# ArchieGertsman/spark-sched-sim

Hardware: AMD Instinct MI355X
Metric: env-steps/sec at 4096 batched envs (TPC-H, 10 exec) (higher is better)
Workload: dtype int64+f64

## Files before the change

include/sss.h:

```cpp
#ifndef SSS_H
#define SSS_H
#include <stddef.h>
#include <stdint.h>

#ifdef __cplusplus
extern "C" {
#endif

typedef struct sss_handle sss_handle;

typedef struct sss_cfg {
  int32_t num_executors;
  int32_t job_arrival_cap;
  int32_t max_jobs;
  int32_t reserved;
  double job_arrival_rate;
  double moving_delay;
  double warmup_delay;
  double beta;
} sss_cfg;

typedef struct sss_dims {
  int32_t num_envs, num_executors, job_cap, stage_stride;
  int32_t node_cap;
// ... 24 lines not shown
  SSS_E_STALLED = 5,
  SSS_E_NO_DURATION = 6,
  SSS_E_INVARIANT = 7,
  SSS_E_NEED_RESET = 8,
  SSS_E_NO_LIMIT = 9,
  SSS_E_CAPACITY = 10
};

int sss_query_dims(const sss_cfg* cfg, const void* pack, size_t pack_bytes, int num_envs, sss_dims* out);

int sss_create(const sss_cfg* cfg, const void* pack, size_t pack_bytes, int num_envs, int device, sss_handle** out);

int sss_bind_buffers(sss_handle* h, const sss_buffers* buffers);

int sss_reset(sss_handle* h, const uint64_t* seeds_dev, const double* time_limits_dev, const uint8_t* mask_dev, void* stream);

#define SSS_SKIP_ENV (-2147483647 - 1)
int sss_step(sss_handle* h, const int32_t* stage_idx_dev, const int32_t* num_exec_dev, int auto_reset, uint64_t seed_stride, void* stream);

int sss_step_bounded(sss_handle* h, const int32_t* stage_idx_dev, const int32_t* num_exec_dev, int auto_reset, uint64_t seed_stride, int max_events,
                     uint8_t* ready_dev, void* stream);

int sss_policy(sss_handle* h, int policy, int param, int32_t* stage_idx_dev, int32_t* num_exec_dev, void* stream);

int sss_rollout(sss_handle* h, int policy, int param, int n_steps, int auto_reset, uint64_t seed_stride, void* stream);

typedef struct sss_decima_graph {
  const uint8_t* active_dev;
  const int64_t* node_off_dev;
  const int64_t* job_off_dev;
  const int64_t* edge_off_dev;
  float num_tasks_scale;
  float work_scale;
  float* x_dev;
  int64_t* node_obs_dev;
  int64_t* node_loc_dev;
  int64_t* node_job_dev;
  int64_t* sched_rank_dev;
  int32_t* gen_dev;
  uint32_t* node_recv_dev;
  uint8_t* stage_mask_dev;
  int64_t* src_dev;
  int64_t* dst_dev;
  int64_t* edge_obs_dev;
  uint32_t* edge_layers_dev;
  int64_t* job_obs_dev;
// ... 333 lines not shown
```

spark_sched_sim_amd/binding.py:

```python
from __future__ import annotations

import ctypes as C
import os.path as osp

CSRC = osp.join(osp.dirname(osp.abspath(__file__)), "csrc")
LIB_NAME = "libsss_hip.so"


class SssCfg(C.Structure):
    _fields_ = [("num_executors", C.c_int32), ("job_arrival_cap", C.c_int32), ("max_jobs", C.c_int32),
                ("reserved", C.c_int32), ("job_arrival_rate", C.c_double), ("moving_delay", C.c_double),
                ("warmup_delay", C.c_double), ("beta", C.c_double)]


class SssDims(C.Structure):
    _fields_ = [("num_envs", C.c_int32), ("num_executors", C.c_int32), ("job_cap", C.c_int32),
                ("stage_stride", C.c_int32), ("node_cap", C.c_int32), ("edge_cap", C.c_int32),
                ("obs_i32", C.c_int32), ("obs_f64", C.c_int32), ("state_bytes", C.c_int64),
                ("env_stride", C.c_int64), ("off_t_arrival", C.c_int64), ("off_t_completed", C.c_int64),
                ("off_jobs", C.c_int64), ("off_active", C.c_int64), ("off_dur_ring", C.c_int64),
                ("job_rec_bytes", C.c_int32), ("hdr_bytes", C.c_int32)]


class SssBuffers(C.Structure):
# ... 109 lines not shown
    _fields_ = [("bits_dev", C.c_void_p), ("n", C.c_int64), ("n_layers", C.c_int32), ("chunk", C.c_int32), ("n_chunks", C.c_int32), ("phase", C.c_int32),
                ("cnt_dev", C.c_void_p), ("off_dev", C.c_void_p), ("base", C.c_int64 * 32), ("out_dev", C.c_void_p)]


class SssReturnsArgs(C.Structure):
    _fields_ = [("T", C.c_int64), ("B", C.c_int64), ("active_dev", C.c_void_p), ("t_before_dev", C.c_void_p), ("t_after_dev", C.c_void_p), ("rewards_dev", C.c_void_p),
                ("beta", C.c_double), ("out_dev", C.c_void_p)]


class SssBaselineArgs(C.Structure):
    _fields_ = [("T", C.c_int64), ("B", C.c_int64), ("R", C.c_int32), ("skip_empty", C.c_int32), ("active_dev", C.c_void_p), ("times_dev", C.c_void_p),
                ("values_dev", C.c_void_p), ("n_dev", C.c_void_p), ("out_dev", C.c_void_p)]


class SssArenaArray(C.Structure):
    _fields_ = [("src_dev", C.c_void_p), ("dst_dev", C.c_void_p), ("elem_bytes", C.c_int32), ("per_row", C.c_int32), ("kind", C.c_int32), ("shift", C.c_int32)]


class SssArenaArgs(C.Structure):
    _fields_ = [("n_arrays", C.c_int32), ("n_obs", C.c_int32), ("totals_dev", C.c_void_p), ("cursor_dev", C.c_void_p), ("capacity", C.c_int64 * 4),
                ("rows_hint", C.c_int64), ("arrays", SssArenaArray * 24)]


EXPORTS = ["sss_query_dims", "sss_create", "sss_bind_buffers", "sss_reset", "sss_step", "sss_step_bounded", "sss_policy", "sss_rollout",
           "sss_decima_graph_build", "sss_decima_layer_lists", "sss_prefix_rows", "sss_decima_policy", "sss_decima_sample", "sss_gnn_launch",
           "sss_linear_wgrad_scratch", "sss_linear_wgrad", "sss_mlp_supported", "sss_mlp_recompute_supported", "sss_mlp_split_supported", "sss_mlp_forward", "sss_mlp_backward", "sss_mlp_wgrad_scratch", "sss_mlp_backward_wgrad", "sss_mlp_wgrad_finish", "sss_collect_step", "sss_gnn_encode", "sss_rows_op", "sss_rows_concat", "sss_segment_categorical", "sss_bit_lists", "sss_arena_append", "sss_discounted_returns", "sss_sequence_baselines", "sss_last_error", "sss_destroy", "sss_abi_sizeof"]
POLICY_IDS = {"fair": 0, "fifo": 1, "hash": 2, "wfair": 3, "sjfcp": 4}
WFAIR_ALPHA_RANGE = (-4, 4)
ABI_STRUCTS = {"sss_cfg": SssCfg, "sss_dims": SssDims, "sss_buffers": SssBuffers, "sss_decima_graph": SssDecimaGraph, "sss_decima_lists": SssDecimaLists,
               "sss_bit_list_args": SssBitListArgs, "sss_gnn_args": SssGnnArgs, "sss_decima_policy_args": SssDecimaPolicyArgs,
               "sss_decima_sample_args": SssDecimaSampleArgs, "sss_gnn_encode_args": SssGnnEncodeArgs, "sss_collect_args": SssCollectArgs,
               "sss_mlp_args": SssMlpArgs, "sss_arena_array": SssArenaArray, "sss_arena_args": SssArenaArgs, "sss_returns_args": SssReturnsArgs,
               "sss_baseline_args": SssBaselineArgs, "sss_rows_args": SssRowsArgs, "sss_concat_part": SssConcatPart, "sss_concat_args": SssConcatArgs, "sss_segcat_args": SssSegcatArgs}


def load_library(path: str | None = None) -> C.CDLL:
    path = path or osp.join(CSRC, LIB_NAME)
    if not osp.exists(path):
        raise RuntimeError(
            f"{path} not found: the HIP extension has not been built "
            "(run `python -c 'import __graft_entry__ as g; g.build()'` or spark_sched_sim_amd/build.py). "
            "There is no CPU fallback.")
    return C.CDLL(path)


class Binding:
    def __init__(self, lib: C.CDLL | None = None):
        self.lib = lib if lib is not None else load_library()
        L = self.lib
        L.sss_query_dims.argtypes = [C.POINTER(SssCfg), C.c_void_p, C.c_size_t, C.c_int, C.POINTER(SssDims)]
        L.sss_create.argtypes = [C.POINTER(SssCfg), C.c_void_p, C.c_size_t, C.c_int, C.c_int, C.POINTER(C.c_void_p)]
        L.sss_bind_buffers.argtypes = [C.c_void_p, C.POINTER(SssBuffers)]
        L.sss_reset.argtypes = [C.c_void_p, C.c_void_p, C.c_void_p, C.c_void_p, C.c_void_p]
        L.sss_step.argtypes = [C.c_void_p, C.c_void_p, C.c_void_p, C.c_int, C.c_uint64, C.c_void_p]
        L.sss_step_bounded.argtypes = [C.c_void_p, C.c_void_p, C.c_void_p, C.c_int, C.c_uint64, C.c_int, C.c_void_p, C.c_void_p]
        L.sss_policy.argtypes = [C.c_void_p, C.c_int, C.c_int, C.c_void_p, C.c_void_p, C.c_void_p]
        L.sss_rollout.argtypes = [C.c_void_p, C.c_int, C.c_int, C.c_int, C.c_int, C.c_uint64, C.c_void_p]
        L.sss_decima_graph_build.argtypes = [C.c_void_p, C.POINTER(SssDecimaGraph), C.c_void_p]
        L.sss_decima_layer_lists.argtypes = [C.c_int, C.POINTER(SssDecimaLists), C.c_void_p]
        L.sss_prefix_rows.argtypes = [C.c_void_p, C.c_int64, C.c_int64, C.c_void_p, C.c_int, C.c_int, C.c_void_p, C.c_void_p, C.c_void_p, C.c_void_p]
        L.sss_decima_policy.argtypes = [C.c_void_p, C.POINTER(SssDecimaPolicyArgs), C.c_void_p]
        L.sss_decima_sample.argtypes = [C.c_int, C.c_int, C.POINTER(SssDecimaSampleArgs), C.c_void_p]
        L.sss_gnn_launch.argtypes = [C.c_int, C.POINTER(SssGnnArgs), C.c_void_p]
        L.sss_linear_wgrad_scratch.argtypes = [C.c_int, C.c_int]
        L.sss_linear_wgrad_scratch.restype = C.c_int64
        L.sss_linear_wgrad.argtypes = [C.c_void_p, C.c_int64, C.c_void_p, C.c_int64, C.c_int64, C.c_int, C.c_int, C.c_void_p, C.c_void_p, C.c_void_p, C.c_void_p]
        L.sss_gnn_encode.argtypes = [C.POINTER(SssGnnEncodeArgs), C.c_void_p]
        L.sss_collect_step.argtypes = [C.POINTER(SssCollectArgs), C.c_int, C.c_void_p]
        L.sss_mlp_supported.argtypes = [C.c_int] * 5
        L.sss_mlp_recompute_supported.argtypes = [C.c_int]
        L.sss_mlp_split_supported.argtypes = [C.c_int]
        L.sss_mlp_forward.argtypes = [C.POINTER(SssMlpArgs), C.c_void_p]
        L.sss_mlp_backward.argtypes = [C.POINTER(SssMlpArgs), C.c_void_p]
        L.sss_mlp_wgrad_scratch.argtypes = [C.c_int]
        L.sss_mlp_wgrad_scratch.restype = C.c_int64
        L.sss_mlp_backward_wgrad.argtypes = [C.POINTER(SssMlpArgs), C.c_void_p, C.c_void_p]
        L.sss_mlp_wgrad_finish.argtypes = [C.c_int] + [C.c_void_p] * 8
        L.sss_discounted_returns.argtypes = [C.POINTER(SssReturnsArgs), C.c_void_p]
        L.sss_sequence_baselines.argtypes = [C.POINTER(SssBaselineArgs), C.c_void_p]
        L.sss_bit_lists.argtypes = [C.POINTER(SssBitListArgs), C.c_void_p]
# ... 1 lines not shown
        L.sss_rows_op.argtypes = [C.POINTER(SssRowsArgs), C.c_void_p]
        L.sss_rows_concat.argtypes = [C.POINTER(SssConcatArgs), C.c_void_p]
        L.sss_segment_categorical.argtypes = [C.POINTER(SssSegcatArgs), C.c_int, C.c_void_p]
        L.sss_last_error.restype = C.c_char_p
        L.sss_destroy.argtypes = [C.c_void_p]
        L.sss_abi_sizeof.argtypes = [C.c_char_p]
        self.check_abi()

    def check_abi(self) -> None:
        bad = [(name, C.sizeof(cls), self.lib.sss_abi_sizeof(name.encode())) for name, cls in ABI_STRUCTS.items()
               if C.sizeof(cls) != self.lib.sss_abi_sizeof(name.encode())]
        if bad:
            raise RuntimeError("binding / library mismatch (struct, sizeof in binding.py, sizeof in the library): " + ", ".join(map(str, bad)))

    def check(self, rc: int) -> None:
        if rc != 0:
            raise ValueError(f"sss error {rc}: {self.lib.sss_last_error().decode()}")

    def query_dims(self, cfg: SssCfg, pack: bytes, num_envs: int) -> SssDims:
        d = SssDims()
        self.check(self.lib.sss_query_dims(C.byref(cfg), pack, len(pack), num_envs, C.byref(d)))
        return d

    def create(self, cfg: SssCfg, pack: bytes, num_envs: int, device: int) -> C.c_void_p:
        h = C.c_void_p()
        self.check(self.lib.sss_create(C.byref(cfg), pack, len(pack), num_envs, device, C.byref(h)))
        return h


def device_of(dev):
    import contextlib

    import torch
    dev = torch.device(dev)
    return torch.cuda.device(dev) if dev.type == "cuda" else contextlib.nullcontext()
```

spark_sched_sim_amd/csrc/sss_hip_sim.hip:

```cpp
#include <hip/hip_runtime.h>

#include "sss_sim.h"
#include "sss_narrow.h"

int sss_narrow_hot_bytes() { return (int)sizeof(SssHot); }
int sss_narrow_static_lds_bytes() { return SSS_STATIC_LDS_BYTES; }

int sss_narrow_launch_reset(const SssKernelArgs& a, int num_envs, const uint64_t* seeds, const double* tl, const uint8_t* mask, void* stream) {
  hipLaunchKernelGGL(sss_reset_kernel, dim3(num_envs), dim3(64), (size_t)a.P.pool_bytes, (hipStream_t)stream, a, seeds, tl, mask);
  return (int)hipGetLastError();
}
int sss_narrow_launch_step_bounded(const SssKernelArgs& a, int num_envs, const int32_t* stage_idx, const int32_t* num_exec, int auto_reset, uint64_t seed_stride,
                                   int budget, uint8_t* ready, void* stream) {
  hipLaunchKernelGGL(sss_step_bounded_kernel, dim3(num_envs), dim3(64), (size_t)a.P.pool_bytes, (hipStream_t)stream, a, stage_idx, num_exec, auto_reset, seed_stride,
                     budget, ready);
  return (int)hipGetLastError();
}
int sss_narrow_launch_step(const SssKernelArgs& a, int num_envs, const int32_t* stage_idx, const int32_t* num_exec, int auto_reset, uint64_t seed_stride,
                           void* stream) {
  hipLaunchKernelGGL(sss_step_kernel, dim3(num_envs), dim3(64), (size_t)a.P.pool_bytes, (hipStream_t)stream, a, stage_idx, num_exec, auto_reset, seed_stride);
  return (int)hipGetLastError();
}
int sss_narrow_launch_policy(const SssKernelArgs& a, int num_envs, int policy, int param, int32_t* stage_idx, int32_t* num_exec, void* stream) {
  hipLaunchKernelGGL(sss_policy_kernel, dim3(num_envs), dim3(64), (size_t)a.P.pool_bytes, (hipStream_t)stream, a, policy, param, stage_idx, num_exec);
  return (int)hipGetLastError();
}
int sss_narrow_launch_rollout(const SssKernelArgs& a, int num_envs, int policy, int param, int n_steps, int auto_reset, uint64_t seed_stride, void* stream) {
  if (policy >= SSS_POLICY_WFAIR)
    hipLaunchKernelGGL(sss_rollout_heur_kernel, dim3(num_envs), dim3(64), (size_t)a.P.pool_bytes, (hipStream_t)stream, a, policy, param, n_steps, auto_reset, seed_stride);
  else
    hipLaunchKernelGGL(sss_rollout_kernel, dim3(num_envs), dim3(64), (size_t)a.P.pool_bytes, (hipStream_t)stream, a, policy, param, n_steps, auto_reset, seed_stride);
  return (int)hipGetLastError();
}

#ifdef SSS_EVPROF3
extern "C" int sss_debug_prof(unsigned long long* out64) {
  if (hipMemcpyFromSymbol(out64, HIP_SYMBOL(g_prof3), sizeof(unsigned long long) * 96) != hipSuccess) return -1;
  static const unsigned long long zeros[96] = {0};
  return hipMemcpyToSymbol(HIP_SYMBOL(g_prof3), zeros, sizeof(zeros)) == hipSuccess ? 0 : -1;
}
extern "C" int sss_debug_prof_min(unsigned long long min_step_ticks) {
  return hipMemcpyToSymbol(HIP_SYMBOL(g_prof3_min), &min_step_ticks, sizeof(min_step_ticks)) == hipSuccess ? 0 : -1;
}
// ... 2 lines not shown
```

spark_sched_sim_amd/csrc/sss_hip_wide.hip:

```cpp
#define SSS_WIDE 1
#include <hip/hip_runtime.h>

#include "sss_sim.h"
#include "sss_wide.h"

int sss_wide_hot_bytes() { return (int)sizeof(SssHot); }
int sss_wide_static_lds_bytes() { return SSS_STATIC_LDS_BYTES; }

int sss_wide_launch_reset(const SssKernelArgs& a, int num_envs, const uint64_t* seeds, const double* tl, const uint8_t* mask, void* stream) {
  hipLaunchKernelGGL(sss_reset_kernel_wide, dim3(num_envs), dim3(64), (size_t)a.P.pool_bytes, (hipStream_t)stream, a, seeds, tl, mask);
  return (int)hipGetLastError();
}
int sss_wide_launch_step_bounded(const SssKernelArgs& a, int num_envs, const int32_t* stage_idx, const int32_t* num_exec, int auto_reset, uint64_t seed_stride,
                                 int budget, uint8_t* ready, void* stream) {
  hipLaunchKernelGGL(sss_step_bounded_kernel_wide, dim3(num_envs), dim3(64), (size_t)a.P.pool_bytes, (hipStream_t)stream, a, stage_idx, num_exec, auto_reset,
                     seed_stride, budget, ready);
  return (int)hipGetLastError();
}
int sss_wide_launch_step(const SssKernelArgs& a, int num_envs, const int32_t* stage_idx, const int32_t* num_exec, int auto_reset, uint64_t seed_stride,
                         void* stream) {
  hipLaunchKernelGGL(sss_step_kernel_wide, dim3(num_envs), dim3(64), (size_t)a.P.pool_bytes, (hipStream_t)stream, a, stage_idx, num_exec, auto_reset, seed_stride);
  return (int)hipGetLastError();
}
int sss_wide_launch_policy(const SssKernelArgs& a, int num_envs, int policy, int param, int32_t* stage_idx, int32_t* num_exec, void* stream) {
  hipLaunchKernelGGL(sss_policy_kernel_wide, dim3(num_envs), dim3(64), (size_t)a.P.pool_bytes, (hipStream_t)stream, a, policy, param, stage_idx, num_exec);
  return (int)hipGetLastError();
}
int sss_wide_launch_rollout(const SssKernelArgs& a, int num_envs, int policy, int param, int n_steps, int auto_reset, uint64_t seed_stride, void* stream) {
  if (policy >= SSS_POLICY_WFAIR)
    hipLaunchKernelGGL(sss_rollout_heur_kernel_wide, dim3(num_envs), dim3(64), (size_t)a.P.pool_bytes, (hipStream_t)stream, a, policy, param, n_steps, auto_reset, seed_stride);
  else
    hipLaunchKernelGGL(sss_rollout_kernel_wide, dim3(num_envs), dim3(64), (size_t)a.P.pool_bytes, (hipStream_t)stream, a, policy, param, n_steps, auto_reset, seed_stride);
  return (int)hipGetLastError();
}

#ifdef SSS_EVPROF3
extern "C" int sss_debug_prof_wide(unsigned long long* out64) {
  if (hipMemcpyFromSymbol(out64, HIP_SYMBOL(g_prof3), sizeof(unsigned long long) * 96) != hipSuccess) return -1;
  static const unsigned long long zeros[96] = {0};
  return hipMemcpyToSymbol(HIP_SYMBOL(g_prof3), zeros, sizeof(zeros)) == hipSuccess ? 0 : -1;
}
extern "C" int sss_debug_prof_min_wide(unsigned long long min_step_ticks) {
  return hipMemcpyToSymbol(HIP_SYMBOL(g_prof3_min), &min_step_ticks, sizeof(min_step_ticks)) == hipSuccess ? 0 : -1;
}
#endif
```

spark_sched_sim_amd/csrc/sss_host.h:

```cpp
#pragma once
#include <math.h>
#include <stdio.h>
#include <stdlib.h>
#include <string.h>

#include <string>
#include <vector>

#include "../../include/sss.h"
#include "sss_layout.h"
#include "sss_train.h"
#include "sss_rows.h"
#include "sss_narrow.h"
#include "sss_wide.h"

static bool sss_is_wide(int num_executors) { return num_executors > 64; }
static int sss_hot_bytes(int num_executors) { return sss_is_wide(num_executors) ? sss_wide_hot_bytes() : sss_narrow_hot_bytes(); }

static thread_local std::string g_sss_err;
static int sss_fail(int code, const std::string& msg) {
  g_sss_err = msg;
  return code;
}

// ... 60 lines not shown
      }
      if (!moved) break;
    }
    for (int i = 0; i < n; i++) best = dist[i] > best ? dist[i] : best;
  }
  return best;
}

struct sss_handle {
  sss_cfg cfg;
  SssPackHost ph;
  int max_dag_depth;
  SssLayout L;
  SssBuffers B;
  bool bound;
  int device;
  void* pack_dev;
  void* zig_dev;
  void* eff_dev;
  void* jump_dev;
  void* common_dev;
  SssParams P;
  SssPackDev pk;
};

static int sss_validate(const sss_cfg* cfg, const void* pack, size_t pack_bytes, int num_envs, SssPackHost* ph, int* J_cap) {
  if (!cfg) return sss_fail(-1, "cfg is NULL");
  if (int prc = sss_pack_parse((const uint8_t*)pack, pack_bytes, ph))
    return sss_fail(-2, prc == -2   ? "workload pack: a stage has a negative task count (a count beyond int32 wrapped when the pack was written)"
                        : prc == -3 ? "workload pack: negative task duration (a duration beyond int32 milliseconds wrapped when the pack was written, or the trace set holds one)"
                        : prc == -4 ? "workload pack: a duration list descriptor points outside the duration pool or holds 2^30 or more entries"
                                    : "workload pack is malformed (expected SSSPACK2, n_queries x n_sizes templates, <= 64 stages/job, <= 255 edges/job, <= 16 executor levels)");
  if (num_envs < 1) return sss_fail(-3, "num_envs must be >= 1");
  if (cfg->num_executors < 1 || cfg->num_executors > SSS_MAX_EXEC_ANY) return sss_fail(-4, "num_executors must be in [1, 128]");
  int cap = cfg->job_arrival_cap > 0 ? cfg->job_arrival_cap : 0;
  int jc = cfg->max_jobs > 0 ? cfg->max_jobs : cap;
  if (jc <= 0) return sss_fail(-5, "max_jobs is required when job_arrival_cap is None");
  if (cap > jc) return sss_fail(-5, "max_jobs is smaller than job_arrival_cap");
  if (jc > SSS_MAX_JOBS) return sss_fail(-5, "job capacity above 1024 is not supported by this build");
  if (!(cfg->job_arrival_rate > 0)) return sss_fail(-6, "job_arrival_rate must be > 0");
  if (!(cfg->beta >= 0)) return sss_fail(-6, "beta must be >= 0");
  *J_cap = jc;
  return 0;
}

static std::vector<int32_t> sss_build_eff(const uint8_t* pack, const SssPackHost& ph, const int8_t lvl_of[8], double warmup_delay) {
  const uint32_t* keymask = (const uint32_t*)(pack + ph.sec_off[7]);
// ... 239 lines not shown
    return sss_fail(-13, "copying the duration descriptors to the device failed");
  }
  std::vector<uint8_t> common = sss_build_common_pool(cfg->num_executors);
  h->common_dev = be_alloc(common.size());
  if (!h->common_dev || be_h2d(h->common_dev, common.data(), common.size())) {
    sss_destroy(h);
    return sss_fail(-11, "device allocation failed");
  }
  pk.eff = (const int32_t*)h->eff_dev;
  pk.eff0 = pk.eff + (size_t)ph.total_stages * 8 * 3 * 4;
  pk.pcg_jump = (const uint64_t*)h->jump_dev;
  pk.lvl_thr = (const uint64_t*)h->jump_dev + jump_words;
  pk.common_pool = (const uint8_t*)h->common_dev;
  h->pk = pk;
  *out = h;
  return 0;
}

extern "C" int sss_bind_buffers(sss_handle* h, const sss_buffers* b) {
  if (!h || !b) return sss_fail(-1, "NULL argument");
  if (!b->state_dev || !b->nodes_dev || !b->edge_links_dev || !b->dag_ptr_dev || !b->exec_supplies_dev || !b->obs_i32_dev || !b->obs_f64_dev)
    return sss_fail(-20, "every buffer in sss_buffers must be provided");
  if (((uintptr_t)b->state_dev) & 255) return sss_fail(-21, "state_dev must be 256-byte aligned");
  h->B.state = b->state_dev, h->B.nodes = b->nodes_dev, h->B.edge_links = b->edge_links_dev, h->B.dag_ptr = b->dag_ptr_dev;
  h->B.exec_supplies = b->exec_supplies_dev, h->B.obs_i32 = b->obs_i32_dev, h->B.obs_f64 = b->obs_f64_dev;
  h->B.gen = h->bound ? h->B.gen + 1 : 1, h->B.gen_pad = 0;
  h->bound = true;
  return 0;
}

static SssKernelArgs sss_args(const sss_handle* h) {
  SssKernelArgs a;
  a.L = h->L, a.B = h->B, a.P = h->P, a.pk = h->pk;
  return a;
}

extern "C" int sss_reset(sss_handle* h, const uint64_t* seeds_dev, const double* time_limits_dev, const uint8_t* mask_dev, void* stream) {
  if (!h || !seeds_dev) return sss_fail(-1, "NULL argument");
  if (!h->bound) return sss_fail(-22, "sss_bind_buffers has not been called");
  BeDeviceGuard guard(h->device);
  const SssKernelArgs ka = sss_args(h);
  if (int rc = sss_is_wide(h->L.E) ? sss_wide_launch_reset(ka, h->L.num_envs, seeds_dev, time_limits_dev, mask_dev, stream)
                                   : be_launch_reset(ka, h->L.num_envs, seeds_dev, time_limits_dev, mask_dev, stream)) return sss_fail(-30, std::string("reset launch failed: ") + be_error(rc));
  return 0;
}

extern "C" int sss_step(sss_handle* h, const int32_t* stage_idx_dev, const int32_t* num_exec_dev, int auto_reset, uint64_t seed_stride, void* stream) {
  if (!h || !stage_idx_dev || !num_exec_dev) return sss_fail(-1, "NULL argument");
  if (!h->bound) return sss_fail(-22, "sss_bind_buffers has not been called");
  BeDeviceGuard guard(h->device);
  const SssKernelArgs ka = sss_args(h);
  if (int rc = sss_is_wide(h->L.E) ? sss_wide_launch_step(ka, h->L.num_envs, stage_idx_dev, num_exec_dev, auto_reset, seed_stride, stream)
                                   : be_launch_step(ka, h->L.num_envs, stage_idx_dev, num_exec_dev, auto_reset, seed_stride, stream)) return sss_fail(-30, std::string("step launch failed: ") + be_error(rc));
  return 0;
}

extern "C" int sss_step_bounded(sss_handle* h, const int32_t* stage_idx_dev, const int32_t* num_exec_dev, int auto_reset, uint64_t seed_stride, int max_events,
                                uint8_t* ready_dev, void* stream) {
  if (!h || !stage_idx_dev || !num_exec_dev || !ready_dev) return sss_fail(-1, "NULL argument");
  if (!h->bound) return sss_fail(-22, "sss_bind_buffers has not been called");
  if (max_events < 1) return sss_fail(-35, "sss_step_bounded: max_events must be at least 1");
  BeDeviceGuard guard(h->device);
  const SssKernelArgs ka = sss_args(h);
  if (int rc = sss_is_wide(h->L.E) ? sss_wide_launch_step_bounded(ka, h->L.num_envs, stage_idx_dev, num_exec_dev, auto_reset, seed_stride, max_events, ready_dev, stream)
                                   : be_launch_step_bounded(ka, h->L.num_envs, stage_idx_dev, num_exec_dev, auto_reset, seed_stride, max_events, ready_dev, stream))
    return sss_fail(-30, std::string("step launch failed: ") + be_error(rc));
  return 0;
}

static int sss_check_policy(int policy, int param) {
  if (policy < 0 || policy > 4) return sss_fail(-23, "unknown policy");
  if (policy == 3 && (param < -4 || param > 4)) return sss_fail(-23, "weighted fair: alpha (param) must be in [-4, 4], got " + std::to_string(param));
  return 0;
}

extern "C" int sss_policy(sss_handle* h, int policy, int param, int32_t* stage_idx_dev, int32_t* num_exec_dev, void* stream) {
  if (!h || !stage_idx_dev || !num_exec_dev) return sss_fail(-1, "NULL argument");
  if (!h->bound) return sss_fail(-22, "sss_bind_buffers has not been called");
  BeDeviceGuard guard(h->device);
  if (int rc = sss_check_policy(policy, param)) return rc;
  const SssKernelArgs ka = sss_args(h);
  if (int rc = sss_is_wide(h->L.E) ? sss_wide_launch_policy(ka, h->L.num_envs, policy, param, stage_idx_dev, num_exec_dev, stream)
                                   : be_launch_policy(ka, h->L.num_envs, policy, param, stage_idx_dev, num_exec_dev, stream)) return sss_fail(-30, std::string("policy launch failed: ") + be_error(rc));
  return 0;
}

extern "C" int sss_rollout(sss_handle* h, int policy, int param, int n_steps, int auto_reset, uint64_t seed_stride, void* stream) {
  if (!h) return sss_fail(-1, "NULL argument");
  if (!h->bound) return sss_fail(-22, "sss_bind_buffers has not been called");
  BeDeviceGuard guard(h->device);
  if (int rc = sss_check_policy(policy, param)) return rc;
  if (n_steps < 0) return sss_fail(-24, "n_steps must be >= 0");
  const SssKernelArgs ka = sss_args(h);
  if (int rc = sss_is_wide(h->L.E) ? sss_wide_launch_rollout(ka, h->L.num_envs, policy, param, n_steps, auto_reset, seed_stride, stream)
                                   : be_launch_rollout(ka, h->L.num_envs, policy, param, n_steps, auto_reset, seed_stride, stream)) return sss_fail(-30, std::string("rollout launch failed: ") + be_error(rc));
  return 0;
}

extern "C" int sss_decima_graph_build(sss_handle* h, const sss_decima_graph* g, void* stream) {
  if (!h || !g) return sss_fail(-1, "NULL argument");
  if (!h->bound) return sss_fail(-22, "sss_bind_buffers has not been called");
  BeDeviceGuard guard(h->device);
  if (!g->node_off_dev || !g->job_off_dev || !g->edge_off_dev || !g->x_dev || !g->node_obs_dev || !g->node_loc_dev || !g->node_job_dev ||
      !g->sched_rank_dev || !g->gen_dev || !g->node_recv_dev || !g->stage_mask_dev || !g->src_dev || !g->dst_dev || !g->edge_obs_dev ||
      !g->edge_layers_dev || !g->job_obs_dev || !g->job_cap_dev || !g->job_first_dev || !g->obs_depth_dev ||
      !g->job_nodes_dev || !g->out_start_dev || !g->out_deg_dev || !g->layer_cnt_dev)
    return sss_fail(-1, "NULL argument");
  if ((int64_t)8 * h->L.n_cap + (int64_t)8 * (h->L.J_cap + 1) > 65536 || h->L.n_cap > 65535 || h->L.ed_cap > 65535 || h->max_dag_depth > 24)
    return sss_fail(-25, "node / edge capacity too large for the Decima graph kernel's LDS working set, or a job template deeper than 24 DAG layers");
  SssDecimaArgs d;
  d.active = g->active_dev, d.node_off = g->node_off_dev, d.job_off = g->job_off_dev, d.edge_off = g->edge_off_dev;
// ... 425 lines not shown
```

spark_sched_sim_amd/csrc/sss_narrow.h:

```cpp
#pragma once
#include <stdint.h>

#include "sss_layout.h"

int sss_narrow_hot_bytes();
int sss_narrow_static_lds_bytes();
int sss_narrow_launch_reset(const SssKernelArgs& a, int num_envs, const uint64_t* seeds, const double* tl, const uint8_t* mask, void* stream);
int sss_narrow_launch_step_bounded(const SssKernelArgs& a, int num_envs, const int32_t* stage_idx, const int32_t* num_exec, int auto_reset, uint64_t seed_stride,
                                   int budget, uint8_t* ready, void* stream);
int sss_narrow_launch_step(const SssKernelArgs& a, int num_envs, const int32_t* stage_idx, const int32_t* num_exec, int auto_reset, uint64_t seed_stride, void* stream);
int sss_narrow_launch_policy(const SssKernelArgs& a, int num_envs, int policy, int param, int32_t* stage_idx, int32_t* num_exec, void* stream);
int sss_narrow_launch_rollout(const SssKernelArgs& a, int num_envs, int policy, int param, int n_steps, int auto_reset, uint64_t seed_stride, void* stream);
```

spark_sched_sim_amd/csrc/sss_sim.h:

```cpp
#pragma once
#ifdef SSS_WIDE
#define SSS_KNAME(name) name##_wide
#else
#define SSS_KNAME(name) name
#endif
#include "../../include/sss.h"
#include "sss_layout.h"
#include <wave_rt.h>


struct alignas(16) SssScratch {
  uint8_t pool8[8];
  uint8_t pool8b[8];
  uint64_t rng_buf[64];
  int32_t rng_pos, pad0_[3];
  uint8_t setA[SSS_SET_TABLE];
  uint8_t setB[SSS_SET_TABLE];
  int32_t f_done, f_scan, f_round_continues;
  int32_t m_n_active, m_src_job;
  int32_t n_old_active;
  int32_t events_this_step;
  int32_t events_at_launch;
  int32_t pending_free;
  int32_t pinned_job;
// ... 564 lines not shown
    } \
    write_observation(a.L, a.B, env, reward); \
    wave_sync(); \
  } \
  env_end(base); \
  prof3_flush();

#ifdef __HIP__
#define SSS_ROLLOUT_HEURISTICS false
#else
#define SSS_ROLLOUT_HEURISTICS true
#endif
SSS_KERNEL void SSS_KNAME(sss_rollout_kernel)(SssKernelArgs a, int policy, int param, int n_steps, int auto_reset, uint64_t seed_stride) {
  ROLLOUT_BODY(SSS_ROLLOUT_HEURISTICS)
}
#ifdef __HIP__
SSS_KERNEL void SSS_KNAME(sss_rollout_heur_kernel)(SssKernelArgs a, int policy, int param, int n_steps, int auto_reset, uint64_t seed_stride) {
  ROLLOUT_BODY(true)
}
#endif
#undef ROLLOUT_BODY
#undef SSS_ROLLOUT_HEURISTICS

#undef H
#undef FAIL
#undef CHECK
```

spark_sched_sim_amd/csrc/sss_wide.h:

```cpp
#pragma once
#include <stdint.h>

#include "sss_layout.h"

int sss_wide_hot_bytes();
int sss_wide_static_lds_bytes();
int sss_wide_launch_reset(const SssKernelArgs& a, int num_envs, const uint64_t* seeds, const double* tl, const uint8_t* mask, void* stream);
int sss_wide_launch_step_bounded(const SssKernelArgs& a, int num_envs, const int32_t* stage_idx, const int32_t* num_exec, int auto_reset, uint64_t seed_stride,
                                 int budget, uint8_t* ready, void* stream);
int sss_wide_launch_step(const SssKernelArgs& a, int num_envs, const int32_t* stage_idx, const int32_t* num_exec, int auto_reset, uint64_t seed_stride, void* stream);
int sss_wide_launch_policy(const SssKernelArgs& a, int num_envs, int policy, int param, int32_t* stage_idx, int32_t* num_exec, void* stream);
int sss_wide_launch_rollout(const SssKernelArgs& a, int num_envs, int policy, int param, int n_steps, int auto_reset, uint64_t seed_stride, void* stream);
```

spark_sched_sim_amd/vec_env.py:

```python
from __future__ import annotations

import ctypes as C
from typing import Any, Sequence

import numpy as np
import torch

from . import workload
from .binding import ERROR_NAMES, POLICY_IDS, WFAIR_ALPHA_RANGE, Binding, SssBuffers, SssCfg, SssDecimaGraph, SssDecimaLists, device_of

OBS_FIELDS = ("n_nodes", "n_edges", "n_jobs", "n_schedulable", "num_committable_execs", "source_job_idx",
              "terminated", "err")
NUM_NODE_FEATURES = 3


class BatchedObs(dict):
    """dict of device tensors; rows beyond n_nodes[i] / n_edges[i] / n_jobs[i] of env i are padding.

    keys: nodes f32[B, node_cap, 3], edge_links i32[B, edge_cap, 2], dag_ptr i32[B, job_cap+1],
    exec_supplies i32[B, job_cap], plus one i32[B] tensor per OBS_FIELDS entry.
    """


def _mask_u8(mask: torch.Tensor | None) -> torch.Tensor | None:
    if mask is None:
        return None
    if mask.is_contiguous() and mask.dtype in (torch.bool, torch.uint8):
        return mask.view(torch.uint8)
    return mask.to(torch.uint8).contiguous()


class LateHint:
# ... 13 lines not shown

    def read_tagged(self):
        for k in (self.last, 1 - self.last):
            if self.posted[k] and (not self.cuda or self.events[k].query()):
                self.kept = (self.bufs[k].clone(), self.tags[k])
                break
        kept = getattr(self, "kept", None)
        return (kept[0].clone(), kept[1]) if kept is not None else (self.fill.clone(), None)

    def post(self, t: torch.Tensor, tag=None) -> None:
        k = 1 - self.last
        if self.cuda and self.posted[k] and not self.events[k].query():
            return
        self.bufs[k].copy_(t, non_blocking=True)
        if self.cuda:
            self.events[k].record(torch.cuda.current_stream(t.device))
        self.posted[k], self.last, self.tags[k] = True, k, tag


class VecSparkSchedSimEnv:

    def __init__(self, env_cfg: dict[str, Any], num_envs: int, device: str | torch.device = "cuda:0",
                 pack: bytes | None = None, auto_reset: bool = False, seed_stride: int | None = None,
                 _lib: C.CDLL | None = None) -> None:
        self.device = torch.device(device)
        if self.device.type != "cuda" and _lib is None:
            raise RuntimeError("VecSparkSchedSimEnv runs on an AMD GPU (device='cuda:N'); there is no CPU path")
        sampler = env_cfg.get("data_sampler_cls", "TPCHDataSampler")
        if sampler != "TPCHDataSampler":
            raise ValueError(f"'{sampler}' is not a valid data sampler.")
        self.num_envs = int(num_envs)
        self.num_executors = int(env_cfg["num_executors"])
        self.env_cfg = dict(env_cfg)
        self.auto_reset = bool(auto_reset)
        self.seed_stride = int(seed_stride if seed_stride is not None else num_envs)
        self._b = Binding(_lib)
        self._pack = pack if pack is not None else workload.default_pack()
        cap = env_cfg.get("job_arrival_cap")
        self._cfg = SssCfg(self.num_executors, int(cap) if cap else 0, int(env_cfg.get("max_jobs") or 0), 0,
                           float(env_cfg["job_arrival_rate"]), float(env_cfg["moving_delay"]),
                           float(env_cfg["warmup_delay"]), float(env_cfg.get("beta", 0.0)))
        self.dims = self._b.query_dims(self._cfg, self._pack, self.num_envs)
        dev_index = self.device.index or 0
        self._h = self._b.create(self._cfg, self._pack, self.num_envs, dev_index if self.device.type == "cuda" else -1)
        d, B, dev = self.dims, self.num_envs, self.device
        self._state_raw = torch.zeros(d.state_bytes + 256, dtype=torch.uint8, device=dev)
        off = (-self._state_raw.data_ptr()) % 256
        self.state = self._state_raw[off: off + d.state_bytes]
        self.nodes = torch.zeros((B, d.node_cap, NUM_NODE_FEATURES), dtype=torch.float32, device=dev)
        self.edge_links = torch.zeros((B, d.edge_cap, 2), dtype=torch.int32, device=dev)
        self.dag_ptr = torch.zeros((B, d.job_cap + 1), dtype=torch.int32, device=dev)
        self.exec_supplies = torch.zeros((B, d.job_cap), dtype=torch.int32, device=dev)
        self.obs_i32 = torch.zeros((B, d.obs_i32), dtype=torch.int32, device=dev)
        self.obs_f64 = torch.zeros((B, d.obs_f64), dtype=torch.float64, device=dev)
        self.rebind_buffers()
        self._seeds = torch.zeros(B, dtype=torch.int64, device=dev)
        self._tl = torch.full((B,), float("inf"), dtype=torch.float64, device=dev)
        self._mask = torch.ones(B, dtype=torch.uint8, device=dev)
        self._env_view = self.state.view(B, d.env_stride)
        self._act_stage = torch.zeros(B, dtype=torch.int32, device=dev)
        self._act_nexec = torch.ones(B, dtype=torch.int32, device=dev)
        self._closed = False
        self._dg_pool: dict[int, torch.Tensor] = {}
        self._layer_scratch: dict = {}
        self._never = None
        from .workload import pack_max_depth
        self.max_dag_depth = pack_max_depth(self._pack)
        from .spaces import make_action_space, make_observation_space
        self.single_action_space = make_action_space(self.num_executors)
        self.action_space = self.single_action_space
        self.single_observation_space = make_observation_space(self.num_executors, NUM_NODE_FEATURES)
        self.observation_space = self.single_observation_space


    def rebind_buffers(self) -> None:
        bufs = SssBuffers(self.state.data_ptr(), self.nodes.data_ptr(), self.edge_links.data_ptr(),
                          self.dag_ptr.data_ptr(), self.exec_supplies.data_ptr(), self.obs_i32.data_ptr(),
                          self.obs_f64.data_ptr())
        self._b.check(self._b.lib.sss_bind_buffers(self._h, C.byref(bufs)))

    def _stream(self) -> int:
        return torch.cuda.current_stream(self.device).cuda_stream if self.device.type == "cuda" else 0

    def _obs(self) -> BatchedObs:
# ... 22 lines not shown
        B = self.num_envs
        if seed is None:
            seeds = np.random.SeedSequence().generate_state(B, np.uint64) >> np.uint64(1)
        elif isinstance(seed, (int, np.integer)):
            seeds = np.arange(B, dtype=np.uint64) + np.uint64(int(seed))
        else:
            seeds = np.asarray(list(seed), dtype=np.uint64)
            if seeds.shape != (B,):
                raise ValueError("need one seed per env")
        self._seeds.copy_(torch.from_numpy(seeds.view(np.int64)))
        tl = (options or {}).get("time_limit", np.inf)
        tl_arr = np.broadcast_to(np.asarray(tl, dtype=np.float64), (B,)).copy()
        self._tl.copy_(torch.from_numpy(tl_arr))
        mask_ptr = None
        if mask is not None:
            self._mask.copy_(mask.to(torch.uint8))
            mask_ptr = self._mask.data_ptr()
        self._b.check(self._b.lib.sss_reset(self._h, self._seeds.data_ptr(), self._tl.data_ptr(), mask_ptr, self._stream()))
        return self._obs(), {"wall_time": self.obs_f64[:, 1]}

    def step_async(self, stage_idx: torch.Tensor, num_exec: torch.Tensor) -> None:
        assert stage_idx.dtype == torch.int32 and num_exec.dtype == torch.int32
        assert stage_idx.device == self.device and stage_idx.is_contiguous() and num_exec.is_contiguous()
        self._b.check(self._b.lib.sss_step(self._h, stage_idx.data_ptr(), num_exec.data_ptr(), int(self.auto_reset),
                                           self.seed_stride, self._stream()))

    def step_bounded_async(self, stage_idx: torch.Tensor, num_exec: torch.Tensor, max_events: int, ready: torch.Tensor | None = None) -> torch.Tensor:
        assert stage_idx.dtype == torch.int32 and num_exec.dtype == torch.int32
        assert stage_idx.device == self.device and stage_idx.is_contiguous() and num_exec.is_contiguous()
        if ready is None:
            if getattr(self, "_ready", None) is None:
                self._ready = torch.ones(self.num_envs, dtype=torch.uint8, device=self.device)
            ready = self._ready
        assert ready.dtype == torch.uint8 and ready.is_contiguous() and ready.numel() == self.num_envs
        self._b.check(self._b.lib.sss_step_bounded(self._h, stage_idx.data_ptr(), num_exec.data_ptr(), int(self.auto_reset), self.seed_stride, int(max_events),
                                                   ready.data_ptr(), self._stream()))
        return ready

    def step(self, actions):
        if set(actions.keys()) != {"stage_idx", "num_exec"}:
            raise ValueError("invalid action: does not belong to the action space")
        self.step_async(actions["stage_idx"], actions["num_exec"])
        obs = self._obs()
        f64 = self.obs_f64.clone()
        i32 = self.obs_i32[:, 6:8].clone()
        terminated = i32[:, 0] != 0
        if self._never is None or self._never.shape != terminated.shape:
            self._never = torch.zeros_like(terminated)
        return obs, f64[:, 0], terminated, self._never, {"wall_time": f64[:, 1], "err": i32[:, 1]}


    @staticmethod
    def _policy_id(policy: str, param: int) -> int:
        pid = POLICY_IDS[policy]
        lo, hi = WFAIR_ALPHA_RANGE
        if policy == "wfair" and not lo <= int(param) <= hi:
            raise ValueError(f"wfair: alpha (param) must be an integer in [{lo}, {hi}], got {param}")
        return pid

    def policy_actions(self, policy: str = "fair", param: int = 0):
        pid = self._policy_id(policy, param)
        self._b.check(self._b.lib.sss_policy(self._h, pid, int(param), self._act_stage.data_ptr(),
                                             self._act_nexec.data_ptr(), self._stream()))
        return {"stage_idx": self._act_stage, "num_exec": self._act_nexec}

    def rollout(self, policy: str, n_steps: int, param: int = 0) -> None:
        pid = self._policy_id(policy, param)
        self._b.check(self._b.lib.sss_rollout(self._h, pid, int(param), int(n_steps), int(self.auto_reset),
                                              self.seed_stride, self._stream()))

    def decima_graph_on_device(self, active: torch.Tensor | None = None, num_tasks_scale: float = 200.0, work_scale: float = 1e5) -> dict[str, Any]:
        B, dev, d = self.num_envs, self.device, self.dims
        assert self.graph_kernel_fits, "the graph kernel's LDS working set does not fit this node capacity"
        D = self.max_dag_depth
        ws = getattr(self, "_dg_dev", None)
        if ws is None:
            Mc, Ec, Jc = B * d.node_cap, B * d.edge_cap, B * d.job_cap
            e = lambda n, dt, *tail: torch.empty((max(n, 1), *tail), dtype=dt, device=dev)
            ws = self._dg_dev = {
                "x": e(Mc, torch.float32, 5), "node_obs": e(Mc, torch.int64), "node_loc": e(Mc, torch.int64), "node_job": e(Mc, torch.int64),
                "sched_rank": e(Mc, torch.int64), "gen": e(Mc, torch.int32), "node_recv": e(Mc, torch.int32), "stage_mask": e(Mc, torch.bool),
                "src": e(Ec, torch.int64), "dst": e(Ec, torch.int64), "edge_obs": e(Ec, torch.int64), "edge_layers": e(Ec, torch.int32),
                "job_obs": e(Jc, torch.int64), "job_cap": e(Jc, torch.int64), "job_first": e(Jc, torch.int64), "obs_depth": e(B, torch.int32),
                "job_nodes": e(Jc, torch.int64), "out_start": e(Mc, torch.int64), "out_deg": e(Mc, torch.int32),
                "layer_cnt": e(32, torch.int32, B), "sched_list": e(Mc, torch.int64),
                "scan": e(2, torch.int64, 4, B),
# ... 254 lines not shown
```

Before: 24.08 million.

## Fuse next-step heuristic policy into the step kernel with double-buffered actions

Result: no change. 24.31 million (median of 6 runs) (+0.9%).

```diff
diff --git a/include/sss.h b/include/sss.h
--- a/include/sss.h
+++ b/include/sss.h
@@ -70,6 +70,10 @@
                      uint8_t* ready_dev, void* stream);
 
 int sss_policy(sss_handle* h, int policy, int param, int32_t* stage_idx_dev, int32_t* num_exec_dev, void* stream);
+
+int sss_step_policy(sss_handle* h, const int32_t* stage_idx_dev, const int32_t* num_exec_dev, int policy, int param, int32_t* next_stage_idx_dev,
+                    int32_t* next_num_exec_dev, int auto_reset, uint64_t seed_stride, void* stream);
+int sss_precomputed_action(const sss_handle* h, int policy, int param, const int32_t** stage_idx_dev, const int32_t** num_exec_dev);
 
 int sss_rollout(sss_handle* h, int policy, int param, int n_steps, int auto_reset, uint64_t seed_stride, void* stream);
 
diff --git a/spark_sched_sim_amd/binding.py b/spark_sched_sim_amd/binding.py
--- a/spark_sched_sim_amd/binding.py
+++ b/spark_sched_sim_amd/binding.py
@@ -155,10 +155,11 @@
                 ("rows_hint", C.c_int64), ("arrays", SssArenaArray * 24)]
 
 
-EXPORTS = ["sss_query_dims", "sss_create", "sss_bind_buffers", "sss_reset", "sss_step", "sss_step_bounded", "sss_policy", "sss_rollout",
+EXPORTS = ["sss_query_dims", "sss_create", "sss_bind_buffers", "sss_reset", "sss_step", "sss_step_bounded", "sss_policy", "sss_step_policy", "sss_precomputed_action", "sss_rollout",
            "sss_decima_graph_build", "sss_decima_layer_lists", "sss_prefix_rows", "sss_decima_policy", "sss_decima_sample", "sss_gnn_launch",
            "sss_linear_wgrad_scratch", "sss_linear_wgrad", "sss_mlp_supported", "sss_mlp_recompute_supported", "sss_mlp_split_supported", "sss_mlp_forward", "sss_mlp_backward", "sss_mlp_wgrad_scratch", "sss_mlp_backward_wgrad", "sss_mlp_wgrad_finish", "sss_collect_step", "sss_gnn_encode", "sss_rows_op", "sss_rows_concat", "sss_segment_categorical", "sss_bit_lists", "sss_arena_append", "sss_discounted_returns", "sss_sequence_baselines", "sss_last_error", "sss_destroy", "sss_abi_sizeof"]
 POLICY_IDS = {"fair": 0, "fifo": 1, "hash": 2, "wfair": 3, "sjfcp": 4}
+FOLDABLE_POLICY_IDS = (0, 1, 2)
 WFAIR_ALPHA_RANGE = (-4, 4)
 ABI_STRUCTS = {"sss_cfg": SssCfg, "sss_dims": SssDims, "sss_buffers": SssBuffers, "sss_decima_graph": SssDecimaGraph, "sss_decima_lists": SssDecimaLists,
                "sss_bit_list_args": SssBitListArgs, "sss_gnn_args": SssGnnArgs, "sss_decima_policy_args": SssDecimaPolicyArgs,
@@ -189,6 +190,8 @@
         L.sss_step_bounded.argtypes = [C.c_void_p, C.c_void_p, C.c_void_p, C.c_int, C.c_uint64, C.c_int, C.c_void_p, C.c_void_p]
         L.sss_policy.argtypes = [C.c_void_p, C.c_int, C.c_int, C.c_void_p, C.c_void_p, C.c_void_p]
         L.sss_rollout.argtypes = [C.c_void_p, C.c_int, C.c_int, C.c_int, C.c_int, C.c_uint64, C.c_void_p]
+        L.sss_step_policy.argtypes = [C.c_void_p, C.c_void_p, C.c_void_p, C.c_int, C.c_int, C.c_void_p, C.c_void_p, C.c_int, C.c_uint64, C.c_void_p]
+        L.sss_precomputed_action.argtypes = [C.c_void_p, C.c_int, C.c_int, C.POINTER(C.c_void_p), C.POINTER(C.c_void_p)]
         L.sss_decima_graph_build.argtypes = [C.c_void_p, C.POINTER(SssDecimaGraph), C.c_void_p]
         L.sss_decima_layer_lists.argtypes = [C.c_int, C.POINTER(SssDecimaLists), C.c_void_p]
         L.sss_prefix_rows.argtypes = [C.c_void_p, C.c_int64, C.c_int64, C.c_void_p, C.c_int, C.c_int, C.c_void_p, C.c_void_p, C.c_void_p, C.c_void_p]
@@ -236,6 +239,12 @@
         self.check(self.lib.sss_query_dims(C.byref(cfg), pack, len(pack), num_envs, C.byref(d)))
         return d
 
+    def precomputed_action(self, h, policy: int, param: int):
+        si, ne = C.c_void_p(), C.c_void_p()
+        if self.lib.sss_precomputed_action(h, policy, param, C.byref(si), C.byref(ne)) != 1:
+            return None
+        return si.value, ne.value
+
     def create(self, cfg: SssCfg, pack: bytes, num_envs: int, device: int) -> C.c_void_p:
         h = C.c_void_p()
         self.check(self.lib.sss_create(C.byref(cfg), pack, len(pack), num_envs, device, C.byref(h)))
diff --git a/spark_sched_sim_amd/csrc/sss_hip_sim.hip b/spark_sched_sim_amd/csrc/sss_hip_sim.hip
--- a/spark_sched_sim_amd/csrc/sss_hip_sim.hip
+++ b/spark_sched_sim_amd/csrc/sss_hip_sim.hip
@@ -19,6 +19,12 @@
 int sss_narrow_launch_step(const SssKernelArgs& a, int num_envs, const int32_t* stage_idx, const int32_t* num_exec, int auto_reset, uint64_t seed_stride,
                            void* stream) {
   hipLaunchKernelGGL(sss_step_kernel, dim3(num_envs), dim3(64), (size_t)a.P.pool_bytes, (hipStream_t)stream, a, stage_idx, num_exec, auto_reset, seed_stride);
+  return (int)hipGetLastError();
+}
+int sss_narrow_launch_step_policy(const SssKernelArgs& a, int num_envs, const int32_t* stage_idx, const int32_t* num_exec, int auto_reset, uint64_t seed_stride,
+                                  int policy, int param, int32_t* next_stage_idx, int32_t* next_num_exec, void* stream) {
+  hipLaunchKernelGGL(sss_step_policy_kernel, dim3(num_envs), dim3(64), (size_t)a.P.pool_bytes, (hipStream_t)stream, a, stage_idx, num_exec, auto_reset, seed_stride,
+                     policy, param, next_stage_idx, next_num_exec);
   return (int)hipGetLastError();
 }
 int sss_narrow_launch_policy(const SssKernelArgs& a, int num_envs, int policy, int param, int32_t* stage_idx, int32_t* num_exec, void* stream) {
diff --git a/spark_sched_sim_amd/csrc/sss_hip_wide.hip b/spark_sched_sim_amd/csrc/sss_hip_wide.hip
--- a/spark_sched_sim_amd/csrc/sss_hip_wide.hip
+++ b/spark_sched_sim_amd/csrc/sss_hip_wide.hip
@@ -22,6 +22,12 @@
   hipLaunchKernelGGL(sss_step_kernel_wide, dim3(num_envs), dim3(64), (size_t)a.P.pool_bytes, (hipStream_t)stream, a, stage_idx, num_exec, auto_reset, seed_stride);
   return (int)hipGetLastError();
 }
+int sss_wide_launch_step_policy(const SssKernelArgs& a, int num_envs, const int32_t* stage_idx, const int32_t* num_exec, int auto_reset, uint64_t seed_stride,
+                                  int policy, int param, int32_t* next_stage_idx, int32_t* next_num_exec, void* stream) {
+  hipLaunchKernelGGL(sss_step_policy_kernel_wide, dim3(num_envs), dim3(64), (size_t)a.P.pool_bytes, (hipStream_t)stream, a, stage_idx, num_exec, auto_reset, seed_stride,
+                     policy, param, next_stage_idx, next_num_exec);
+  return (int)hipGetLastError();
+}
 int sss_wide_launch_policy(const SssKernelArgs& a, int num_envs, int policy, int param, int32_t* stage_idx, int32_t* num_exec, void* stream) {
   hipLaunchKernelGGL(sss_policy_kernel_wide, dim3(num_envs), dim3(64), (size_t)a.P.pool_bytes, (hipStream_t)stream, a, policy, param, stage_idx, num_exec);
   return (int)hipGetLastError();
diff --git a/spark_sched_sim_amd/csrc/sss_host.h b/spark_sched_sim_amd/csrc/sss_host.h
--- a/spark_sched_sim_amd/csrc/sss_host.h
+++ b/spark_sched_sim_amd/csrc/sss_host.h
@@ -106,7 +106,14 @@
   void* common_dev;
   SssParams P;
   SssPackDev pk;
+  struct {
+    bool valid;
+    int policy, param;
+    const int32_t* stage_idx;
+    const int32_t* num_exec;
+  } pre;
 };
+static void sss_drop_precomputed(sss_handle* h) { h->pre.valid = false; }
 
 static int sss_validate(const sss_cfg* cfg, const void* pack, size_t pack_bytes, int num_envs, SssPackHost* ph, int* J_cap) {
   if (!cfg) return sss_fail(-1, "cfg is NULL");
@@ -392,6 +399,7 @@
   if (!b->state_dev || !b->nodes_dev || !b->edge_links_dev || !b->dag_ptr_dev || !b->exec_supplies_dev || !b->obs_i32_dev || !b->obs_f64_dev)
     return sss_fail(-20, "every buffer in sss_buffers must be provided");
   if (((uintptr_t)b->state_dev) & 255) return sss_fail(-21, "state_dev must be 256-byte aligned");
+  sss_drop_precomputed(h);
   h->B.state = b->state_dev, h->B.nodes = b->nodes_dev, h->B.edge_links = b->edge_links_dev, h->B.dag_ptr = b->dag_ptr_dev;
   h->B.exec_supplies = b->exec_supplies_dev, h->B.obs_i32 = b->obs_i32_dev, h->B.obs_f64 = b->obs_f64_dev;
   h->B.gen = h->bound ? h->B.gen + 1 : 1, h->B.gen_pad = 0;
@@ -407,6 +415,7 @@
 
 extern "C" int sss_reset(sss_handle* h, const uint64_t* seeds_dev, const double* time_limits_dev, const uint8_t* mask_dev, void* stream) {
   if (!h || !seeds_dev) return sss_fail(-1, "NULL argument");
+  sss_drop_precomputed(h);
   if (!h->bound) return sss_fail(-22, "sss_bind_buffers has not been called");
   BeDeviceGuard guard(h->device);
   const SssKernelArgs ka = sss_args(h);
@@ -417,6 +426,7 @@
 
 extern "C" int sss_step(sss_handle* h, const int32_t* stage_idx_dev, const int32_t* num_exec_dev, int auto_reset, uint64_t seed_stride, void* stream) {
   if (!h || !stage_idx_dev || !num_exec_dev) return sss_fail(-1, "NULL argument");
+  sss_drop_precomputed(h);
   if (!h->bound) return sss_fail(-22, "sss_bind_buffers has not been called");
   BeDeviceGuard guard(h->device);
   const SssKernelArgs ka = sss_args(h);
@@ -428,6 +438,7 @@
 extern "C" int sss_step_bounded(sss_handle* h, const int32_t* stage_idx_dev, const int32_t* num_exec_dev, int auto_reset, uint64_t seed_stride, int max_events,
                                 uint8_t* ready_dev, void* stream) {
   if (!h || !stage_idx_dev || !num_exec_dev || !ready_dev) return sss_fail(-1, "NULL argument");
+  sss_drop_precomputed(h);
   if (!h->bound) return sss_fail(-22, "sss_bind_buffers has not been called");
   if (max_events < 1) return sss_fail(-35, "sss_step_bounded: max_events must be at least 1");
   BeDeviceGuard guard(h->device);
@@ -446,6 +457,8 @@
 
 extern "C" int sss_policy(sss_handle* h, int policy, int param, int32_t* stage_idx_dev, int32_t* num_exec_dev, void* stream) {
   if (!h || !stage_idx_dev || !num_exec_dev) return sss_fail(-1, "NULL argument");
+  if (h->pre.valid && (stage_idx_dev == h->pre.stage_idx || stage_idx_dev == h->pre.num_exec || num_exec_dev == h->pre.stage_idx || num_exec_dev == h->pre.num_exec))
+    sss_drop_precomputed(h);
   if (!h->bound) return sss_fail(-22, "sss_bind_buffers has not been called");
   BeDeviceGuard guard(h->device);
   if (int rc = sss_check_policy(policy, param)) return rc;
@@ -455,8 +468,39 @@
   return 0;
 }
 
+extern "C" int sss_step_policy(sss_handle* h, const int32_t* stage_idx_dev, const int32_t* num_exec_dev, int policy, int param, int32_t* next_stage_idx_dev,
+                               int32_t* next_num_exec_dev, int auto_reset, uint64_t seed_stride, void* stream) {
+  if (!h || !stage_idx_dev || !num_exec_dev || !next_stage_idx_dev || !next_num_exec_dev) return sss_fail(-1, "NULL argument");
+  sss_drop_precomputed(h);
+  if (!h->bound) return sss_fail(-22, "sss_bind_buffers has not been called");
+  if (policy < 0 || policy > 2) return sss_fail(-23, "sss_step_policy: policies 0 (fair), 1 (FIFO) and 2 (hash) only; the others take sss_policy + sss_step");
+  if (next_stage_idx_dev == stage_idx_dev || next_stage_idx_dev == num_exec_dev || next_num_exec_dev == stage_idx_dev || next_num_exec_dev == num_exec_dev ||
+      next_stage_idx_dev == next_num_exec_dev)
+    return sss_fail(-39, "sss_step_policy: the next action goes to buffers of its own");
+#ifdef __HIP__
+  BeDeviceGuard guard(h->device);
+  const SssKernelArgs ka = sss_args(h);
+  if (int rc = sss_is_wide(h->L.E) ? sss_wide_launch_step_policy(ka, h->L.num_envs, stage_idx_dev, num_exec_dev, auto_reset, seed_stride, policy, param, next_stage_idx_dev, next_num_exec_dev, stream)
+                                   : sss_narrow_launch_step_policy(ka, h->L.num_envs, stage_idx_dev, num_exec_dev, auto_reset, seed_stride, policy, param, next_stage_idx_dev, next_num_exec_dev, stream))
+    return sss_fail(-30, std::string("step launch failed: ") + be_error(rc));
+  h->pre.valid = true, h->pre.policy = policy, h->pre.param = param, h->pre.stage_idx = next_stage_idx_dev, h->pre.num_exec = next_num_exec_dev;
+  return 0;
+#else
+  (void)auto_reset, (void)seed_stride, (void)stream;
+  return sss_fail(-39, "sss_step_policy: a kernel of the gfx950 build only (here: sss_policy + sss_step)");
+#endif
+}
+
+extern "C" int sss_precomputed_action(const sss_handle* h, int policy, int param, const int32_t** stage_idx_dev, const int32_t** num_exec_dev) {
+  if (!h || !h->pre.valid || h->pre.policy != policy || h->pre.param != param) return 0;
+  if (stage_idx_dev) *stage_idx_dev = h->pre.stage_idx;
+  if (num_exec_dev) *num_exec_dev = h->pre.num_exec;
+  return 1;
+}
+
 extern "C" int sss_rollout(sss_handle* h, int policy, int param, int n_steps, int auto_reset, uint64_t seed_stride, void* stream) {
   if (!h) return sss_fail(-1, "NULL argument");
+  sss_drop_precomputed(h);
   if (!h->bound) return sss_fail(-22, "sss_bind_buffers has not been called");
   BeDeviceGuard guard(h->device);
   if (int rc = sss_check_policy(policy, param)) return rc;
diff --git a/spark_sched_sim_amd/csrc/sss_narrow.h b/spark_sched_sim_amd/csrc/sss_narrow.h
--- a/spark_sched_sim_amd/csrc/sss_narrow.h
+++ b/spark_sched_sim_amd/csrc/sss_narrow.h
@@ -9,5 +9,7 @@
 int sss_narrow_launch_step_bounded(const SssKernelArgs& a, int num_envs, const int32_t* stage_idx, const int32_t* num_exec, int auto_reset, uint64_t seed_stride,
                                    int budget, uint8_t* ready, void* stream);
 int sss_narrow_launch_step(const SssKernelArgs& a, int num_envs, const int32_t* stage_idx, const int32_t* num_exec, int auto_reset, uint64_t seed_stride, void* stream);
+int sss_narrow_launch_step_policy(const SssKernelArgs& a, int num_envs, const int32_t* stage_idx, const int32_t* num_exec, int auto_reset, uint64_t seed_stride,
+                                  int policy, int param, int32_t* next_stage_idx, int32_t* next_num_exec, void* stream);
 int sss_narrow_launch_policy(const SssKernelArgs& a, int num_envs, int policy, int param, int32_t* stage_idx, int32_t* num_exec, void* stream);
 int sss_narrow_launch_rollout(const SssKernelArgs& a, int num_envs, int policy, int param, int n_steps, int auto_reset, uint64_t seed_stride, void* stream);
diff --git a/spark_sched_sim_amd/csrc/sss_sim.h b/spark_sched_sim_amd/csrc/sss_sim.h
--- a/spark_sched_sim_amd/csrc/sss_sim.h
+++ b/spark_sched_sim_amd/csrc/sss_sim.h
@@ -610,6 +610,34 @@
 #undef ROLLOUT_BODY
 #undef SSS_ROLLOUT_HEURISTICS
 
+#ifdef __HIP__
+SSS_KERNEL void SSS_KNAME(sss_step_policy_kernel)(SssKernelArgs a, const int32_t* stage_idx, const int32_t* num_exec, int auto_reset, uint64_t seed_stride, int policy,
+                                                  int param, int32_t* next_stage_idx, int32_t* next_num_exec) {
+  int env = wave_env();
+  uint8_t* base = (uint8_t*)a.B.state + (size_t)env * a.L.env_stride;
+  const bool skipped = stage_idx[env] == SSS_SKIP_ENV;
+  ctx_init();
+  if (skipped) {
+    env_begin_readonly(base);
+  } else {
+    env_begin(base);
+    double reward = 0.0;
+    bool start_next_episode = wave_ballot(auto_reset && g_hot.h.terminated && !g_hot.h.err) != 0;
+    if (start_next_episode)
+      do_reset(a.L, g_hot.h.seed + seed_stride, g_hot.h.time_limit);
+    else
+      reward = do_step(stage_idx[env], num_exec[env]);
+    write_observation(a.L, a.B, env, reward);
+    wave_sync();
+  }
+  int si, ne;
+  run_policy<false>(policy, param, si, ne);
+  if (wave_lane() == 0) next_stage_idx[env] = si, next_num_exec[env] = ne;
+  if (!skipped) env_end(base);
+  prof3_flush();
+}
+#endif
+
 #undef H
 #undef FAIL
 #undef CHECK
diff --git a/spark_sched_sim_amd/csrc/sss_wide.h b/spark_sched_sim_amd/csrc/sss_wide.h
--- a/spark_sched_sim_amd/csrc/sss_wide.h
+++ b/spark_sched_sim_amd/csrc/sss_wide.h
@@ -9,5 +9,7 @@
 int sss_wide_launch_step_bounded(const SssKernelArgs& a, int num_envs, const int32_t* stage_idx, const int32_t* num_exec, int auto_reset, uint64_t seed_stride,
                                  int budget, uint8_t* ready, void* stream);
 int sss_wide_launch_step(const SssKernelArgs& a, int num_envs, const int32_t* stage_idx, const int32_t* num_exec, int auto_reset, uint64_t seed_stride, void* stream);
+int sss_wide_launch_step_policy(const SssKernelArgs& a, int num_envs, const int32_t* stage_idx, const int32_t* num_exec, int auto_reset, uint64_t seed_stride,
+                                  int policy, int param, int32_t* next_stage_idx, int32_t* next_num_exec, void* stream);
 int sss_wide_launch_policy(const SssKernelArgs& a, int num_envs, int policy, int param, int32_t* stage_idx, int32_t* num_exec, void* stream);
 int sss_wide_launch_rollout(const SssKernelArgs& a, int num_envs, int policy, int param, int n_steps, int auto_reset, uint64_t seed_stride, void* stream);
diff --git a/spark_sched_sim_amd/vec_env.py b/spark_sched_sim_amd/vec_env.py
--- a/spark_sched_sim_amd/vec_env.py
+++ b/spark_sched_sim_amd/vec_env.py
@@ -7,7 +7,7 @@
 import torch
 
 from . import workload
-from .binding import ERROR_NAMES, POLICY_IDS, WFAIR_ALPHA_RANGE, Binding, SssBuffers, SssCfg, SssDecimaGraph, SssDecimaLists, device_of
+from .binding import ERROR_NAMES, FOLDABLE_POLICY_IDS, POLICY_IDS, WFAIR_ALPHA_RANGE, Binding, SssBuffers, SssCfg, SssDecimaGraph, SssDecimaLists, device_of
 
 OBS_FIELDS = ("n_nodes", "n_edges", "n_jobs", "n_schedulable", "num_committable_execs", "source_job_idx",
               "terminated", "err")
@@ -67,7 +67,7 @@
 
     def __init__(self, env_cfg: dict[str, Any], num_envs: int, device: str | torch.device = "cuda:0",
                  pack: bytes | None = None, auto_reset: bool = False, seed_stride: int | None = None,
-                 _lib: C.CDLL | None = None) -> None:
+                 _lib: C.CDLL | None = None, fold_policy: bool = True) -> None:
         self.device = torch.device(device)
         if self.device.type != "cuda" and _lib is None:
             raise RuntimeError("VecSparkSchedSimEnv runs on an AMD GPU (device='cuda:N'); there is no CPU path")
@@ -103,8 +103,10 @@
         self._tl = torch.full((B,), float("inf"), dtype=torch.float64, device=dev)
         self._mask = torch.ones(B, dtype=torch.uint8, device=dev)
         self._env_view = self.state.view(B, d.env_stride)
-        self._act_stage = torch.zeros(B, dtype=torch.int32, device=dev)
-        self._act_nexec = torch.ones(B, dtype=torch.int32, device=dev)
+        self._act_pairs = [(torch.zeros(B, dtype=torch.int32, device=dev), torch.ones(B, dtype=torch.int32, device=dev)) for _ in range(2)]
+        self._act_stage, self._act_nexec = self._act_pairs[0]
+        self._act_from = None
+        self.fold_policy = bool(fold_policy) and self.device.type == "cuda"
         self._closed = False
         self._dg_pool: dict[int, torch.Tensor] = {}
         self._layer_scratch: dict = {}
@@ -173,6 +175,12 @@
     def step_async(self, stage_idx: torch.Tensor, num_exec: torch.Tensor) -> None:
         assert stage_idx.dtype == torch.int32 and num_exec.dtype == torch.int32
         assert stage_idx.device == self.device and stage_idx.is_contiguous() and num_exec.is_contiguous()
+        if (self.fold_policy and self._act_from is not None and stage_idx.data_ptr() == self._act_stage.data_ptr()
+                and num_exec.data_ptr() == self._act_nexec.data_ptr() and stage_idx.numel() == self.num_envs):
+            nxt = self._act_pairs[1] if self._act_stage is self._act_pairs[0][0] else self._act_pairs[0]
+            self._b.check(self._b.lib.sss_step_policy(self._h, stage_idx.data_ptr(), num_exec.data_ptr(), self._act_from[0], self._act_from[1],
+                                                      nxt[0].data_ptr(), nxt[1].data_ptr(), int(self.auto_reset), self.seed_stride, self._stream()))
+            return
         self._b.check(self._b.lib.sss_step(self._h, stage_idx.data_ptr(), num_exec.data_ptr(), int(self.auto_reset),
                                            self.seed_stride, self._stream()))
 
@@ -211,8 +219,16 @@
 
     def policy_actions(self, policy: str = "fair", param: int = 0):
         pid = self._policy_id(policy, param)
+        if self.fold_policy:
+            pre = self._b.precomputed_action(self._h, pid, int(param))
+            for pair in self._act_pairs if pre is not None else ():
+                if pre == (pair[0].data_ptr(), pair[1].data_ptr()):
+                    self._act_stage, self._act_nexec = pair
+                    self._act_from = (pid, int(param))
+                    return {"stage_idx": self._act_stage, "num_exec": self._act_nexec}
         self._b.check(self._b.lib.sss_policy(self._h, pid, int(param), self._act_stage.data_ptr(),
                                              self._act_nexec.data_ptr(), self._stream()))
+        self._act_from = (pid, int(param)) if pid in FOLDABLE_POLICY_IDS else None
         return {"stage_idx": self._act_stage, "num_exec": self._act_nexec}
 
     def rollout(self, policy: str, n_steps: int, param: int = 0) -> None:
```
